# astroHaoPeng/gp_algos

Hardware: AMD Instinct MI355X
Metric: GP posterior (mu,var) points/sec at n=8192 fp64 (fit + predict per step) (higher is better)
Workload: dtype f64; 1 GPU; C2: GP regression, ARD-RBF, n=8192 d=8 fp64, Gram + Cholesky + posterior mean/variance at m=65536 test points per GPU; n=8192, d=8, m_per_gpu=65536, parallelism=single GPU

## Files before the change

gp_algos_amd/csrc/gpcore_api.hip:

```cpp
#include "gpcore_internal.h"

#include <algorithm>
#include <atomic>
#include <queue>
#include <functional>
#include <new>
#include <thread>

void gp_prof_begin(gp_ctx *ctx, int cls, hipStream_t s) {
    if (!(ctx->prof_which & (1 << cls))) return;
    hipEvent_t e0, e1;
    if (hipEventCreate(&e0) != hipSuccess || hipEventCreate(&e1) != hipSuccess) return;
    (void)hipEventRecord(e0, s ? s : ctx->stream);
    ctx->prof[cls].ev.push_back(e0);
    ctx->prof[cls].ev.push_back(e1);
}
void gp_prof_end(gp_ctx *ctx, int cls, double work, hipStream_t s) {
    if (!(ctx->prof_which & (1 << cls))) return;
    gp_prof_slot &p = ctx->prof[cls];
    if (p.ev.size() < 2) return;
    (void)hipEventRecord(p.ev.back(), s ? s : ctx->stream);
    p.launches += 1;
    p.work += work;
}
// ... 368 lines not shown
        const double tiles128 = trapezoid_flops(rows - c1, nnext, wcols) / (2.0 * GP_NB * GP_NB * wcols);
        if (count == 1 && tiles128 < small_update_tiles() && small_panel_update())
            gpk_gemm_k128_sub(s, rows - c1, nnext, P, lda, P, lda, A + (size_t)c1 + (size_t)c1 * lda, lda, 1, wcols);
        else
            gpk_gemm_nt(s, rows - c1, nnext, wcols, -1.0, P, lda, P, lda, 1.0, A + (size_t)c1 + (size_t)c1 * lda, lda, 1, 0, bgemm);
        gp_prof_end(ctx, GP_PROF_SYRK, count * trapezoid_flops(rows - c1, nnext, wcols));
    }
    if (side_busy) (void)hipStreamWaitEvent(s, ctx->ev_b, 0);
}

void back_solve_vec(gp_ctx *ctx, const double *L, int np, int ldl, const double *dinv, double *z, double *alpha) {
    hipStream_t s = ctx->stream;
    for (int k = np / GP_NB - 1; k >= 0; --k)
        gpk_bwd_step(s, L, ldl, dinv + (size_t)k * GP_NB * 16, z, alpha, k * GP_NB);
}

int rows_left_min() {
    const char *e = getenv("GPCORE_ROWS_LEFT_MIN");
    const int x = e ? atoi(e) : 0;
    return x > 0 ? x : 192;
}

void build_lw(gp_ctx *ctx, double *Lw, double *scratch, const double *L, int np, int ldl, const double *dinv) {
    hipStream_t s = ctx->stream;
    gpk_lw_transpose(s, scratch, np, L, ldl, np, 1);
    gp_batch bt;
    bt.count = np / GP_NB;
    bt.s0 = (size_t)GP_NB * np;
    bt.s1 = (size_t)GP_NB * (ldl + 1);
    bt.s2 = (size_t)GP_NB * 16;
    bt.tri = 1;
    gp_prof_begin(ctx, GP_PROF_TRSM);
    gpk_trsm_panel128(s, scratch, np, np, L, ldl, dinv, nullptr, nullptr, nullptr, bt);
    gp_prof_end(ctx, GP_PROF_TRSM, (double)np * np / 2.0 * GP_NB);
    gpk_lw_transpose(s, Lw, np, scratch, np, np, 0);
}

void solve_rows_lower(gp_ctx *ctx, double *Vt, int mp, const double *L, int np, int ldl, const double *dinv, double *sumsq,
                      const double *tvec = nullptr, double *dots = nullptr, const double *Lw = nullptr) {
    hipStream_t s = ctx->stream;
    const int nblk = np / GP_NB;
    if (Lw && sumsq && (mp / GP_NB) >= rows_left_min()) {
        for (int i = 0; i < nblk; ++i) {
            const int K = (i + 1) * GP_NB;
            gp_prof_begin(ctx, GP_PROF_GEMM);
            gpk_gemm_nt_rowred(s, mp, GP_NB, K, Vt, mp, Lw + (size_t)i * GP_NB, np, Vt + (size_t)i * GP_NB * mp, mp, sumsq,
                               tvec ? tvec + (size_t)i * GP_NB : nullptr, dots);
            gp_prof_end(ctx, GP_PROF_GEMM, 2.0 * mp * GP_NB * (double)K);
        }
        return;
    }
    const bool right_looking = (mp / GP_NB) < rows_left_min();
    if (right_looking) {
        const int ob_env = gp_env_blocks("GPCORE_ROWS_OUTER");
        const int OB = ob_env ? ob_env : 2 * GP_OUTER;
        for (int c0 = 0; c0 < np; c0 += OB) {
            const int c1 = std::min(np, c0 + OB);
            for (int k0 = c0; k0 < c1; k0 += GP_NB) {
                double *Vk = Vt + (size_t)k0 * mp;
                gp_prof_begin(ctx, GP_PROF_TRSM);
                gpk_trsm_panel128(s, Vk, mp, mp, L + (size_t)k0 + (size_t)k0 * ldl, ldl, dinv + (size_t)(k0 / GP_NB) * GP_NB * 16, sumsq,
                                  tvec ? tvec + k0 : nullptr, dots);
                gp_prof_end(ctx, GP_PROF_TRSM, (double)mp * GP_NB * GP_NB);
                const int rest = c1 - (k0 + GP_NB);
                if (rest > 0) {
                    gp_prof_begin(ctx, GP_PROF_GEMM);
                    gemm_sub_single(s, mp, rest, GP_NB, Vk, mp, L + (size_t)(k0 + GP_NB) + (size_t)k0 * ldl, ldl, Vt + (size_t)(k0 + GP_NB) * mp, mp);
                    gp_prof_end(ctx, GP_PROF_GEMM, 2.0 * mp * (double)rest * GP_NB);
                }
            }
// ... 266 lines not shown
        if (stream) { ctx->stream = static_cast<hipStream_t>(stream); ctx->own_stream = false; }
        else { e = hipStreamCreateWithFlags(&ctx->stream, hipStreamNonBlocking); ctx->own_stream = true; }
    }
    if (e == hipSuccess) {
        int reserved = 32;
        if (const char *rc = getenv("GPCORE_RESERVED_CUS")) reserved = atoi(rc);
        hipError_t em = hipErrorInvalidValue;
        if (reserved > 0 && ctx->num_cu >= 64) {
            const int words = (ctx->num_cu + 31) / 32;
            std::vector<uint32_t> mask(words, 0xFFFFFFFFu);
            if (ctx->num_cu % 32) mask[words - 1] = (1u << (ctx->num_cu % 32)) - 1u;
            for (int i = 0; i < reserved && i < ctx->num_cu; ++i) mask[i / 32] &= ~(1u << (i % 32));
            em = hipExtStreamCreateWithCUMask(&ctx->side, (uint32_t)words, mask.data());
        }
        if (em != hipSuccess) { (void)hipGetLastError(); e = hipStreamCreateWithFlags(&ctx->side, hipStreamNonBlocking); }
    }
    if (e == hipSuccess && !g_child_ctx && gpi_ctx_ep_streams(ctx) != GP_OK) e = hipErrorInvalidValue;
    if (e == hipSuccess) e = hipEventCreateWithFlags(&ctx->ev_a, hipEventDisableTiming);
    if (e == hipSuccess) e = hipEventCreateWithFlags(&ctx->ev_b, hipEventDisableTiming);
    if (const char *la = getenv("GPCORE_LOOKAHEAD")) ctx->lookahead = atoi(la) != 0 ? 1 : 0;
    if (e == hipSuccess) e = hipMalloc(&ctx->d_scalars, sizeof(double) * 256);
    if (e == hipSuccess) e = hipMalloc(&ctx->d_info, sizeof(int) * 8 + sizeof(double) * 64);
    if (e == hipSuccess) e = hipMemset(ctx->d_info, 0, sizeof(int) * 8 + sizeof(double) * 64);
    if (e == hipSuccess && (gpk_init_diag_kernels() != 0 || gpk_init_gemm_kernels() != 0)) e = hipErrorInvalidValue;
    if (e != hipSuccess) { delete ctx; return GP_EHIP; }
    *out = ctx;
    return GP_OK;
}

void gp_ctx_destroy(gp_ctx *ctx) {
    if (!ctx) return;
    (void)hipSetDevice(ctx->device);
    (void)hipStreamSynchronize(ctx->stream);
    for (int c = 0; c < GP_PROF_NCLASSES; ++c)
        for (hipEvent_t e : ctx->prof[c].ev) (void)hipEventDestroy(e);
    ctx_ext *x = ext_of(ctx);
    for (gp_ctx *c : x->children) gp_ctx_destroy(c);
    x->children.clear();
    (void)hipSetDevice(ctx->device);
    for (int i = 0; i < WS_COUNT; ++i) if (x->ws[i].p) (void)hipFree(x->ws[i].p);
    if (x->mega.d_tasks) (void)hipFree(x->mega.d_tasks);
    if (x->mega.d_done) (void)hipFree(x->mega.d_done);
    if (x->mega.d_ctl) (void)hipFree(x->mega.d_ctl);
    if (x->mega.d_sums) (void)hipFree(x->mega.d_sums);
    if (ctx->d_scalars) (void)hipFree(ctx->d_scalars);
    if (ctx->d_info) (void)hipFree(ctx->d_info);
    if (ctx->ev_a) (void)hipEventDestroy(ctx->ev_a);
// ... 423 lines not shown
    double *Vt, *partial, *sumsq;
    GP_TRY(ws_get(ctx, WS_VT, sizeof(double) * (size_t)mp * np, &Vt));
    GP_TRY(ws_get(ctx, WS_PARTIAL, sizeof(double) * (size_t)nchunk * mp, &partial));
    GP_TRY(ws_get(ctx, WS_SUMSQ, sizeof(double) * (size_t)mp, &sumsq));
    if (np > n) gpk_fill(s, Vt + (size_t)n * mp, (size_t)mp * (np - n), 0.0);
    if (mp > m) {
        GP_HIP(ctx, hipMemset2DAsync(Vt + m, (size_t)mp * 8, 0, (size_t)(mp - m) * 8, n, s));
    }
    gp_prof_begin(ctx, GP_PROF_GRAM);
    if (mdl->kind == 1) gpk_co2_gram(s, dXs, m, mdl->dX, n, mdl->theta.data(), 0, Vt, mp, 0, 1, 0.0);
    else gpk_gram_cross(s, dXs, m, ldxs, mdl->dX, n, n, mdl->d, mdl->theta.data(), Vt, mp, gp_gram_flag(ctx), mdl->dcen);
    gp_prof_end(ctx, GP_PROF_GRAM, 8.0 * m * (double)n + 8.0 * (m + n) * mdl->d);
    double *dots = partial;
    GP_HIP(ctx, hipMemsetAsync(sumsq, 0, sizeof(double) * mp, s));
    GP_HIP(ctx, hipMemsetAsync(dots, 0, sizeof(double) * mp, s));
    const double *Lw = nullptr;
    const bool use_lw = [] { const char *e = getenv("GPCORE_POSTERIOR_LW"); return !e || atoi(e) != 0; }();
    if (use_lw && mp / GP_NB >= rows_left_min()) {
        if (!mdl->dLw) {
            hipError_t e = hipMalloc(&mdl->dLw, sizeof(double) * (size_t)np * np);
            if (e != hipSuccess) { mdl->dLw = nullptr; GP_SET_ERR(ctx, "hipMalloc(Lw, n=%d) failed: %s", n, hipGetErrorString(e)); return GP_ENOMEM; }
        }
        if (!mdl->lw_valid) {
            double *scratch;
            GP_TRY(ws_get(ctx, WS_D, sizeof(double) * (size_t)np * np, &scratch));
            build_lw(ctx, mdl->dLw, scratch, mdl->dL, np, mdl->ldl, mdl->ddinv);
            mdl->lw_valid = true;
        }
        Lw = mdl->dLw;
    }
    solve_rows_lower(ctx, Vt, mp, mdl->dL, np, mdl->ldl, mdl->ddinv, sumsq, mdl->dtmp, dots, Lw);
    GP_HIP(ctx, hipMemcpyAsync(dmean, dots, sizeof(double) * m, hipMemcpyDeviceToDevice, s));
    if (dvar) {
        const double sf = mdl->theta[0], sn = mdl->kind == 1 ? 0.0 : mdl->theta[mdl->d + 1];
        gpk_var_finish(s, dvar, sumsq, m, mdl->kind == 1 ? gpk_co2_kss(mdl->theta.data()) : sf * sf + sn * sn);
    }
    if (vt_out) *vt_out = Vt;
    if (mp_out) *mp_out = mp;
    GP_LAUNCH_CHECK(ctx);
    return GP_OK;
}

static int predict_batch_cap() {
    static const int cap = [] { const char *e = getenv("GPCORE_PREDICT_BATCH"); int v = e ? atoi(e) : 0; return v >= GP_NB ? v / GP_NB * GP_NB : 131072; }();
    return cap;
}

gp_status gp_predict_dev(gp_model *mdl, const double *dXs, int m, int ldxs, double *dmean, double *dvar) {
    if (!mdl) return GP_EINVAL;
// ... 649 lines not shown
```

gp_algos_amd/csrc/gpcore_ep.hip:

```cpp
#include "gpcore_internal.h"
#include "dpp_tile.h"
#include "trsm_tile.h"

#include <algorithm>
#include <atomic>
#include <chrono>
#include <cmath>
#include <new>
#include <thread>
#include <vector>

constexpr int EP_OUTER = 4 * GP_NB;

struct gp_ep {
    gp_ctx *ctx = nullptr;
    int n = 0, np = 0;
    double *K = nullptr;
    double *Sig = nullptr;
    double *Sig2 = nullptr;
    double *L = nullptr;
    int ldl = 0;
    double *dinv = nullptr;
    double *S = nullptr;
    double *Sc = nullptr;
// ... 1385 lines not shown
    GP_REQUIRE(ctx, ep->dX, "classifier was built from a Gram matrix");
    GP_REQUIRE(ctx, dXs && dprob && m >= 0 && ldxs >= m && batch_rows >= 0, "bad arguments");
    GP_REQUIRE(ctx, ep->sweeps > 0, "classifier not trained: run gp_ep_sweep first");
    if (m == 0) return GP_OK;
    GP_HIP(ctx, hipSetDevice(ctx->device));
    hipStream_t s = ctx->stream;
    const int n = ep->n, np = ep->np, d = ep->d;
    int batch = batch_rows > 0 ? std::max(GP_NB, batch_rows / GP_NB * GP_NB)
                               : (int)std::min<size_t>(131072, std::max<size_t>(GP_NB, (((size_t)32 << 30) / ((size_t)np * 8)) / GP_NB * GP_NB));
    batch = std::min(batch, gp_pad(m));
    double *Vt, *partial, *sumsq, *fm;
    GP_TRY(gpi_ws_get(ctx, WS_VT, sizeof(double) * (size_t)batch * np, &Vt));
    GP_TRY(gpi_ws_get(ctx, WS_PARTIAL, sizeof(double) * (size_t)16 * np, &partial));
    GP_TRY(gpi_ws_get(ctx, WS_SUMSQ, sizeof(double) * (size_t)batch, &sumsq));
    GP_TRY(gpi_ws_get(ctx, WS_B, sizeof(double) * (size_t)batch, &fm));
    const double *Lw = nullptr;
    if (batch / GP_NB >= gpi_rows_left_min()) {
        if (!ep->Lw) {
            hipError_t e = hipMalloc(&ep->Lw, sizeof(double) * (size_t)np * np);
            if (e != hipSuccess) { (void)hipGetLastError(); ep->Lw = nullptr; GP_SET_ERR(ctx, "hipMalloc(Lw, n=%d) failed: %s", n, hipGetErrorString(e)); return GP_ENOMEM; }
            ep->lw_valid = false;
        }
        if (!ep->lw_valid) {
            double *scratch;
            GP_TRY(gpi_ws_get(ctx, WS_D, sizeof(double) * (size_t)np * np, &scratch));
            gpi_build_lw(ctx, ep->Lw, scratch, ep->L, np, ep->ldl, ep->dinv);
            ep->lw_valid = true;
        }
        Lw = ep->Lw;
    }
    double *w = ep->tmp2();
    gpk_gemv_rows(s, ep->K, n, n, np, ep->nu(), ep->tmp1(), partial, 16);
    hipLaunchKernelGGL(vec_mul_kernel, g1(n), dim3(256), 0, s, ep->tmp1(), ep->tmp1(), ep->st(), n);
    gpi_forward_solve_vec(ctx, ep->L, np, ep->ldl, ep->dinv, ep->tmp1(), ep->tmp2());
    gpi_back_solve_vec(ctx, ep->L, np, ep->ldl, ep->dinv, ep->tmp2(), ep->tmp1());
    hipLaunchKernelGGL(ep_w_kernel, g1(np), dim3(256), 0, s, w, ep->nu(), ep->st(), ep->tmp1(), n, np);
    const double sf = ep->theta[0], sn = ep->theta[d + 1];
    const double kss = sf * sf + sn * sn;
    for (int lo = 0; lo < m; lo += batch) {
        const int mb = std::min(batch, m - lo), mp = gp_pad(mb);
        gp_prof_begin(ctx, GP_PROF_GRAM);
        gpk_gram_cross(s, dXs + lo, mb, ldxs, ep->dX, n, n, d, ep->theta.data(), Vt, mp, gp_gram_flag(ctx), ep->dcen);
        gp_prof_end(ctx, GP_PROF_GRAM, 8.0 * mb * (double)n + 8.0 * (mb + n) * d);
        hipLaunchKernelGGL(ep_mean_scale_kernel, dim3(mp / GP_NB), dim3(64 * EP_MS_CHUNKS), 0, s, Vt, mp, np, mb, n, w, ep->st(), fm);
        GP_HIP(ctx, hipMemsetAsync(sumsq, 0, sizeof(double) * mp, s));
        gpi_solve_rows_lower(ctx, Vt, mp, ep->L, np, ep->ldl, ep->dinv, sumsq, nullptr, nullptr, Lw);
        hipLaunchKernelGGL(ep_prob_latent_kernel, g1(mb), dim3(256), 0, s, dprob + lo, dfmean ? dfmean + lo : nullptr,
                           dfvar ? dfvar + lo : nullptr, fm, sumsq, kss, mb);
    }
// ... 242 lines not shown
```

gp_algos_amd/csrc/gpcore_internal.h:

```cpp
#pragma once
#include <hip/hip_runtime.h>
#include <cstdint>
#include <cstdio>
#include <cstring>
#include <cstdlib>
#include <cmath>
#include <functional>
#include <vector>

#include "../../include/gpcore.h"

constexpr int GP_NB = 128;
constexpr int GP_BK = 16;
constexpr int GP_OUTER = 512;
static inline int gp_pad(int n) { return (n + GP_NB - 1) / GP_NB * GP_NB; }
static inline int gp_env_blocks(const char *name) {
    const char *e = getenv(name);
    const int v = e ? atoi(e) : 0;
    return (v >= GP_NB && v % GP_NB == 0) ? v : 0;
}

struct gp_prof_slot {
    int64_t launches = 0;
    double work = 0.0;
// ... 45 lines not shown
#define GP_SET_ERR(ctx, ...) do { if (ctx) snprintf((ctx)->err, sizeof((ctx)->err), __VA_ARGS__); } while (0)
#define GP_HIP(ctx, call) do { hipError_t e_ = (call); if (e_ != hipSuccess) { \
    GP_SET_ERR(ctx, "%s:%d %s -> %s", __FILE__, __LINE__, #call, hipGetErrorString(e_)); return GP_EHIP; } } while (0)
#define GP_LAUNCH_CHECK(ctx) GP_HIP(ctx, hipGetLastError())
#define GP_REQUIRE(ctx, cond, msg) do { if (!(cond)) { GP_SET_ERR(ctx, "invalid argument: %s", msg); return GP_EINVAL; } } while (0)
#define GP_TRY(call) do { gp_status s_ = (call); if (s_ != GP_OK) return s_; } while (0)

void gp_prof_begin(gp_ctx *ctx, int cls, hipStream_t s = nullptr);
void gp_prof_end(gp_ctx *ctx, int cls, double work, hipStream_t s = nullptr);

struct gp_batch {
    int count = 1;
    size_t s0 = 0, s1 = 0, s2 = 0;
    size_t s3 = 0, s4 = 0, s5 = 0;
    int tri = 0;
};

void gpk_gemm_nt(hipStream_t s, int M, int N, int K, double alpha, const double *A, int lda, const double *B, int ldb,
                 double beta, double *C, int ldc, int lower, int ktri = 0, gp_batch bt = gp_batch(),
                 const double *Cin = nullptr, int ldcin = 0,
                 int *uflag = nullptr);
void gpk_gemm_k128_sub(hipStream_t s, int M, int N, const double *A, int lda, const double *B, int ldb, double *C, int ldc, int lower, int K = 128);
void gpk_gemm_nt_rowred(hipStream_t s, int M, int N, int K, const double *A, int lda, const double *B, int ldb, double *C, int ldc,
                        double *sumsq, const double *tvec, double *dots);
void gpk_gram_sym(hipStream_t s, const double *X, int n, int d, int ldx, const double *theta, double *K, int ldk, int full, double extra_diag, int *far_flag,
                  const double *center = nullptr);
void gpk_centroid(hipStream_t s, const double *X, int n, int d, int ldx, double *c);
void gpk_dgram_sym(hipStream_t s, const double *X, int n, int d, int ldx, const double *theta, int pos, double *D, int ldd);
void gpk_gram_cross(hipStream_t s, const double *Xs, int m, int ldxs, const double *X, int n, int ldx, int d, const double *theta, double *Ks, int ldks, int *far_flag,
                    const double *center = nullptr);
inline int *gp_gram_flag(gp_ctx *ctx) { return ctx->d_info + 4; }
inline double *gp_gram_center(gp_ctx *ctx) { return reinterpret_cast<double *>(ctx->d_info + 8); }
void gpk_co2_gram(hipStream_t s, const double *xr, int nr, const double *xc, int nc, const double *theta, int pos, double *K, int ldk, int sym,
                  int full, double extra);
void gpk_co2_trace(hipStream_t s, int n, const double *alpha, const double *Kinv, int ldk, const double *D, int ldd, double *partial, double *out);
double gpk_co2_kss(const double *theta);
void gpk_pad_identity(hipStream_t s, double *A, int n, int np, int lda);
void gpk_zero_upper(hipStream_t s, double *A, int n, int lda);
void gpk_fill(hipStream_t s, double *p, size_t count, double v);
void gpk_trsm_panel_upper(hipStream_t s, double *X, int M, int ldx, const double *Ukk, int ldu);
void gpk_transpose(hipStream_t s, double *dst, int ldd, const double *src, int lds, int rows, int cols);
void gpk_lw_transpose(hipStream_t s, double *dst, int ldd, const double *src, int lds, int np, int stage);
void gpk_set_identity(hipStream_t s, double *A, int n, int lda);
void gpk_set_identity_upper(hipStream_t s, double *A, int n, int lda);
void gpk_add_diag(hipStream_t s, double *A, int n, int lda, double v);
void gpk_lml_grad_traces(hipStream_t s, const double *X, int n, int d, int ldx, const double *theta, const double *alpha,
                         const double *Kinv, int ldk, double *partials, double *out);
int gpk_lml_grad_partials_size(int n, int d);
void gpk_gemv_panel_sub(hipStream_t s, const double *A, int M, int lda, const double *x, double *y);
void gpk_gemv_rows(hipStream_t s, const double *Ks, int m, int n, int ldks, const double *alpha, double *out, double *partial, int nchunk, int upper_blocks = 0);
void gpk_lml(hipStream_t s, const double *L, int n, int ldl, const double *t, double *out);
void gpk_var_finish(hipStream_t s, double *var, const double *sumsq, int m, double kss);
size_t gpk_predict_grad_partials(int m, int n, int d);
void gpk_predict_grad(hipStream_t s, const double *Wt, int ldw, const double *Xs, int m, int ldxs, const double *X, int n, int ldx, int d,
                      const double *theta, const double *alpha, double *partials, double *gmean, double *gvar, int ldg);
void gpk_copy_2d(hipStream_t s, double *dst, int ldd, const double *src, int lds, int rows, int cols);
double gpk_probe_mfma(hipStream_t s, int num_cu, int waves_per_simd, double *clock_mhz, double *cycles_per_mfma);
int gpk_init_diag_kernels();
int gpk_init_gemm_kernels();
void gpk_potrf_diag128(hipStream_t s, double *A, int lda, double *dinv_k, int *d_info, int base, gp_batch bt = gp_batch());
void gpk_chol_mega(hipStream_t s, int num_cu, double *A, int lda, double *dinv, int *d_info, const int *tasks, int ntasks, int *done, int *counter,
                   int epoch, int *err, double *sums, unsigned long long *stamps = nullptr);
void gpk_ep_link(hipStream_t s, double *X, int ldx, const double *Lmat, const double *dinv, const double *tvec, double *dots, double *X2,
                 const double *cs2, double *D, int ldd);
void gpk_trsm_panel128(hipStream_t s, double *X, int M, int ldx, const double *Lkk, int ldl, const double *dinv_k, double *sumsq,
                       const double *tvec = nullptr, double *dots = nullptr, gp_batch bt = gp_batch(),
                       double *X2 = nullptr, const double *cs2 = nullptr);
void gpk_fwd_step(hipStream_t s, const double *L, int ldl, const double *dinv_k, double *t, double *sol, int k0, int r);
void gpk_bwd_step(hipStream_t s, const double *L, int ldl, const double *dinv_k, double *t, double *sol, int k0);
void gpk_tile_inverses(hipStream_t s, const double *L, int np, int ldl, double *dinv);
void gpk_copy_strided(hipStream_t s, double *dst, size_t dst_stride, const double *src, size_t src_stride, int count);

enum { WS_VT = 0, WS_PARTIAL, WS_SUMSQ, WS_A, WS_B, WS_C, WS_D, WS_E, WS_F, WS_G, WS_H, WS_COUNT };
gp_status gpi_ws_get(gp_ctx *ctx, int slot, size_t bytes, double **out);
gp_status gpi_upload_2d(gp_ctx *ctx, double *dst, int ldd, const double *src, int lds, int rows, int cols);
gp_status gpi_download_2d(gp_ctx *ctx, double *dst, int ldd, const double *src, int lds, int rows, int cols);
gp_status gpi_read_info(gp_ctx *ctx, int *info);
gp_ctx *gpi_child_ctx(gp_ctx *ctx, int k);
gp_status gpi_model_alpha(gp_model *m, double *dst);
gp_status gpi_model_alloc(gp_ctx *ctx, int n, int d, bool has_x, gp_model **out);
gp_status gpi_lbfgs_maximize(gp_ctx *ctx, int P, int nparams, const double *theta0, int max_iter, int history, int NC,
                             const std::function<gp_status(const double *, int, double *, double *, int *)> &evaluate,
// ... 17 lines not shown
```

gp_algos_amd/csrc/kernels_chol.hip:

```cpp
#include "gpcore_internal.h"

namespace {

constexpr int NB = GP_NB;

__global__ __launch_bounds__(256) void gemv_panel_sub_kernel(const double *__restrict__ A, int M, int lda,
                                                             const double *__restrict__ x, double *__restrict__ y) {
    __shared__ double xs[NB];
    if (threadIdx.x < NB) xs[threadIdx.x] = x[threadIdx.x];
    __syncthreads();
    const int p = blockIdx.x * 256 + threadIdx.x;
    if (p >= M) return;
    double acc = 0.0;
#pragma unroll 8
    for (int k = 0; k < NB; ++k) acc = fma(A[p + (size_t)k * lda], xs[k], acc);
    y[p] -= acc;
}

__global__ __launch_bounds__(256) void gemv_rows_kernel(const double *__restrict__ Ks, int m, int n, int ldks,
                                                        const double *__restrict__ alpha, double *__restrict__ partial,
                                                        int nchunk, int upper_blocks) {
    const int i = blockIdx.x * 256 + threadIdx.x;
    const int ch = blockIdx.y;
    const int per = (n + nchunk - 1) / nchunk;
// ... 61 lines not shown
            for (int c2 = 0; c2 < cc; ++c2) acc[c2] = fma(-x, uc[c2], acc[c2]);
        }
#pragma unroll
        for (int cc = 0; cc < 16; ++cc) xr[(size_t)(cb + cc) * ldx] = acc[cc];
    }
}

__global__ __launch_bounds__(256) void transpose_kernel(double *__restrict__ dst, int ldd, const double *__restrict__ src, int lds,
                                                        int rows, int cols) {
    __shared__ double t[64][65];
    const int r0 = blockIdx.x * 64, c0 = blockIdx.y * 64;
    const int tx = threadIdx.x & 63, ty = threadIdx.x >> 6;
    for (int q = ty; q < 64; q += 4) {
        int r = r0 + tx, c = c0 + q;
        t[q][tx] = (r < rows && c < cols) ? src[r + (size_t)c * lds] : 0.0;
    }
    __syncthreads();
    for (int q = ty; q < 64; q += 4) {
        int c = c0 + tx, r = r0 + q;
        if (r < rows && c < cols) dst[c + (size_t)r * ldd] = t[tx][q];
    }
}

__device__ __forceinline__ void tile_transpose_64(double (*t)[65], double *__restrict__ out, int ldo, int ro, int co,
                                                  const double *__restrict__ in, int ldi, int ri, int ci, double sign) {
    const int tx = threadIdx.x & 63, ty = threadIdx.x >> 6;
    __syncthreads();
    for (int q = ty; q < 64; q += 4) t[q][tx] = in[(ri + tx) + (size_t)(ci + q) * ldi];
    __syncthreads();
    for (int q = ty; q < 64; q += 4) out[(ro + tx) + (size_t)(co + q) * ldo] = sign * t[tx][q];
}
__device__ __forceinline__ void tile_fill_64(double *__restrict__ out, int ldo, int ro, int co, bool identity) {
    const int tx = threadIdx.x & 63, ty = threadIdx.x >> 6;
    for (int q = ty; q < 64; q += 4) out[(ro + tx) + (size_t)(co + q) * ldo] = (identity && tx == q) ? 1.0 : 0.0;
}

__global__ __launch_bounds__(256) void lw_transpose_kernel(double *__restrict__ dst, int ldd, const double *__restrict__ src, int lds, int stage) {
    __shared__ double t[64][65];
    const int ti = blockIdx.x, tj = blockIdx.y;
    if (tj > ti) return;
    const bool same128 = (ti >> 1) == (tj >> 1);
    if (stage) {
        if (!same128) tile_transpose_64(t, dst, ldd, tj * 64, ti * 64, src, lds, ti * 64, tj * 64, -1.0);
        else if (ti == tj) tile_fill_64(dst, ldd, ti * 64, ti * 64, true);
        else { tile_fill_64(dst, ldd, tj * 64, ti * 64, false); tile_fill_64(dst, ldd, ti * 64, tj * 64, false); }
    } else {
        tile_transpose_64(t, dst, ldd, ti * 64, tj * 64, src, lds, tj * 64, ti * 64, 1.0);
        if (same128 && ti != tj) tile_transpose_64(t, dst, ldd, tj * 64, ti * 64, src, lds, ti * 64, tj * 64, 1.0);
    }
}

__global__ void add_diag_kernel(double *A, int n, int lda, double v) {
    const int i = blockIdx.x * blockDim.x + threadIdx.x;
    if (i < n) A[i + (size_t)i * lda] += v;
}
__global__ void set_identity_kernel(double *A, int n, int lda) {
    size_t total = (size_t)n * n;
    for (size_t e = blockIdx.x * (size_t)blockDim.x + threadIdx.x; e < total; e += (size_t)gridDim.x * blockDim.x) {
        int i = (int)(e % n), j = (int)(e / n);
        A[i + (size_t)j * lda] = (i == j) ? 1.0 : 0.0;
    }
}

__global__ void set_identity_upper_kernel(double *A, int n, int lda) {
    for (int j = blockIdx.y; j < n; j += gridDim.y) {
        const int rows = (j & ~127) + 128;
        for (int i = blockIdx.x * blockDim.x + threadIdx.x; i < rows; i += gridDim.x * blockDim.x) A[i + (size_t)j * lda] = (i == j) ? 1.0 : 0.0;
    }
}

constexpr int TR_T = 64, TR_DC = 8, TR_DMAX = 64;
struct TraceParams { double inv_ls2[TR_DMAX]; };
// ... 191 lines not shown
}

struct TraceScale { double s[TR_DMAX + 2]; };
__global__ __launch_bounds__(256) void lml_grad_reduce_kernel(const double *__restrict__ partials, int nblocks, int P, TraceScale sc,
                                                              double *__restrict__ out) {
    __shared__ double red[256];
    const int p = blockIdx.x;
    double acc = 0.0;
    for (int b = threadIdx.x; b < nblocks; b += 256) acc += partials[(size_t)b * P + p];
    double tot = block_sum_256(acc, red);
    if (threadIdx.x == 0) out[p] = sc.s[p] * tot;
}

}

void gpk_trsm_panel_upper(hipStream_t s, double *X, int M, int ldx, const double *Ukk, int ldu) {
    if (M <= 0) return;
    hipLaunchKernelGGL(trsm_panel_upper_kernel, dim3((M + 63) / 64), dim3(64), 0, s, X, M, ldx, Ukk, ldu);
}
void gpk_transpose(hipStream_t s, double *dst, int ldd, const double *src, int lds, int rows, int cols) {
    if (rows <= 0 || cols <= 0) return;
    hipLaunchKernelGGL(transpose_kernel, dim3((rows + 63) / 64, (cols + 63) / 64), dim3(256), 0, s, dst, ldd, src, lds, rows, cols);
}
void gpk_lw_transpose(hipStream_t s, double *dst, int ldd, const double *src, int lds, int np, int stage) {
    hipLaunchKernelGGL(lw_transpose_kernel, dim3(np / 64, np / 64), dim3(256), 0, s, dst, ldd, src, lds, stage);
}
void gpk_add_diag(hipStream_t s, double *A, int n, int lda, double v) {
    if (n > 0) hipLaunchKernelGGL(add_diag_kernel, dim3((n + 255) / 256), dim3(256), 0, s, A, n, lda, v);
}
void gpk_set_identity(hipStream_t s, double *A, int n, int lda) {
    hipLaunchKernelGGL(set_identity_kernel, dim3(1024), dim3(256), 0, s, A, n, lda);
}
void gpk_set_identity_upper(hipStream_t s, double *A, int n, int lda) {
    hipLaunchKernelGGL(set_identity_upper_kernel, dim3(4, n < 65535 ? n : 65535), dim3(256), 0, s, A, n, lda);
}
constexpr int TR_MAX_WG = 768;
int gpk_lml_grad_partials_size(int n, int d) {
    (void)n;
    return TR_MAX_WG * (d + 2);
}
void gpk_lml_grad_traces(hipStream_t s, const double *X, int n, int d, int ldx, const double *theta, const double *alpha,
                         const double *Kinv, int ldk, double *partials, double *out) {
    TraceParams prm;
    TraceScale sc;
    const double sf = theta[0], sn = theta[d + 1];
    for (int k = 0; k < TR_DMAX; ++k) prm.inv_ls2[k] = 0.0;
    for (int k = 0; k < TR_DMAX + 2; ++k) sc.s[k] = 0.0;
    sc.s[0] = sf;
// ... 29 lines not shown
```

gp_algos_amd/csrc/kernels_gemm.hip:

```cpp
#include <type_traits>
#include "gpcore_internal.h"
#include <algorithm>

typedef double double4_t __attribute__((ext_vector_type(4)));
typedef double double2_t __attribute__((ext_vector_type(2)));

namespace {

constexpr int TM = 128, TN = 128, TK = GP_BK;
constexpr int LDS_STRIDE = TM + 16;

__device__ __forceinline__ void tile_coords_lower(int t, int nbm, int nbn, int &bi, int &bj) {
    constexpr int G = 4;
    for (int c0 = 0; c0 < nbn; c0 += G) {
        const int w = (nbn - c0 < G) ? nbn - c0 : G;
        const int head = w * (w + 1) / 2;
        const int total = head + (nbm - c0 - w) * w;
        if (t < total) {
            int r, c;
            if (t < head) {
                r = 0;
                while ((r + 1) * (r + 2) / 2 <= t) ++r;
                c = t - r * (r + 1) / 2;
            } else {
// ... 168 lines not shown
            rsq[mt] += __shfl_xor(rsq[mt], 16, 64);
            rsq[mt] += __shfl_xor(rsq[mt], 32, 64);
            rdt[mt] += __shfl_xor(rdt[mt], 16, 64);
            rdt[mt] += __shfl_xor(rdt[mt], 32, 64);
            if (fk == 0) {
                red[(wave >> 1) * TM + wm + mt * 16 + fr] = rsq[mt];
                red[(NW / 2 + (wave >> 1)) * TM + wm + mt * 16 + fr] = rdt[mt];
            }
        }
        __syncthreads();
        if (tid < TM) {
            double a = 0.0, b = 0.0;
#pragma unroll
            for (int g = 0; g < NW / 2; ++g) { a += red[g * TM + tid]; b += red[(NW / 2 + g) * TM + tid]; }
            rr.sumsq[row0 + tid] += a;
            if (rr.dots) rr.dots[row0 + tid] += b;
        }
    }
}

constexpr int FM = 256, FSTRIDE = FM + 16;
template <int LOWER, int HAS_BETA, int RR, int WV = 16>
__global__ __launch_bounds__(WV * 64, 1) void gemm_fused_kernel(int M, int N, int K, double alpha, const double *A, int lda, const double *B, int ldb,
                                                            double beta, double *C, int ldc, gp_batch bt, gemm_rowred rr) {
    extern __shared__ __attribute__((aligned(16))) double fsm[];
    double *As = fsm;
    double *Bs = fsm + 2 * TK * FSTRIDE;
    const int nbm = M / FM, nbn = N / TN;
    int bi, bj;
    if (LOWER) {
        int t = blockIdx.x;
        bi = 0;
        for (;;) {
            const int cnt = (2 * bi + 2 < nbn) ? 2 * bi + 2 : nbn;
            if (t < cnt) break;
            t -= cnt;
            ++bi;
        }
        bj = t;
    } else {
        const int nwg = gridDim.x, id = blockIdx.x;
        const int q = nwg >> 3, r = nwg & 7, xcd = id & 7;
        const int swz = (xcd < r ? xcd * (q + 1) : r * (q + 1) + (xcd - r) * q) + (id >> 3);
        bi = swz % nbm;
        bj = swz / nbm;
    }
    A += (size_t)blockIdx.y * bt.s0;
// ... 4 lines not shown
    constexpr int NT = (WV == 16) ? 2 : 4;
    const int wm = (wave & 3) * 64, wn = (wave >> 2) * (NT * 16);
    const int fr = lane & 15, fk = lane >> 4;
    const double *Asrc = A + row0 + lane * 2 + (size_t)wave * lda;
    const double *Bsrc = B + col0 + lane * 2 + (size_t)wave * ldb;
    auto stage = [&](int buf, int kt) {
        const size_t koff = (size_t)kt * TK;
#pragma unroll
        for (int q = 0; q < TK / WV; ++q) {
            const int kr = wave + WV * q;
            __builtin_amdgcn_global_load_lds(Asrc + (koff + WV * q) * lda, As + (buf * TK + kr) * FSTRIDE, 16, 0, 0);
            __builtin_amdgcn_global_load_lds(Asrc + 128 + (koff + WV * q) * lda, As + (buf * TK + kr) * FSTRIDE + 128, 16, 0, 0);
            __builtin_amdgcn_global_load_lds(Bsrc + (koff + WV * q) * ldb, Bs + (buf * TK + kr) * LDS_STRIDE, 16, 0, 0);
        }
    };
    double4_t acc[NT][4];
#pragma unroll
    for (int a = 0; a < NT; ++a)
#pragma unroll
        for (int b = 0; b < 4; ++b) acc[a][b] = (double4_t){0.0, 0.0, 0.0, 0.0};
    const int KT = K / TK;
    if (KT > 0) stage(0, 0);
    __syncthreads();
    for (int kt = 0; kt < KT; ++kt) {
        const int cur = kt & 1;
        if (kt + 1 < KT) stage(cur ^ 1, kt + 1);
        const double *Ac = As + cur * TK * FSTRIDE + wm + fr;
        const double *Bc = Bs + cur * TK * LDS_STRIDE + wn + fr;
#pragma unroll
        for (int ks = 0; ks < TK / 4; ++ks) {
            double af[4], bf[NT];
#pragma unroll
            for (int t = 0; t < 4; ++t) af[t] = Ac[(ks * 4 + fk) * FSTRIDE + t * 16];
#pragma unroll
            for (int t = 0; t < NT; ++t) bf[t] = Bc[(ks * 4 + fk) * LDS_STRIDE + t * 16];
#pragma unroll
            for (int nt = 0; nt < NT; ++nt)
#pragma unroll
                for (int mt = 0; mt < 4; ++mt)
                    acc[nt][mt] = __builtin_amdgcn_mfma_f64_16x16x4f64(bf[nt], af[mt], acc[nt][mt], 0, 0, 0);
        }
        __syncthreads();
    }
    const bool diag = LOWER && (row0 < col0 + TN);
    double rsq[4] = {0.0, 0.0, 0.0, 0.0}, rdt[4] = {0.0, 0.0, 0.0, 0.0};
    auto epilogue = [&](auto masked_t) {
        constexpr bool MASKED = decltype(masked_t)::value;
#pragma unroll
        for (int nt = 0; nt < NT; ++nt) {
            double cv[4][4];
            if (HAS_BETA) {
#pragma unroll
                for (int r = 0; r < 4; ++r) {
                    const int n = col0 + wn + nt * 16 + fk + 4 * r;
#pragma unroll
                    for (int mt = 0; mt < 4; ++mt) {
                        const int m = row0 + wm + mt * 16 + fr;
                        cv[r][mt] = (MASKED && m < n) ? 0.0 : C[m + (size_t)n * ldc];
                    }
                }
            }
#pragma unroll
            for (int r = 0; r < 4; ++r) {
                const int n = col0 + wn + nt * 16 + fk + 4 * r;
                const double tn = (RR && rr.dots) ? rr.tvec[n] : 0.0;
// ... 155 lines not shown
    if (uflag) ntiles += 2;
    if (ktri) {
        if (!lower || M != N) return;
        int most = 0;
        for (int x = 0; x < 8; ++x) {
            int cnt = 0;
            for (int r = x; r < M / TM; r += 8) cnt += (r + 1) * bt.count;
            most = cnt > most ? cnt : most;
        }
        ntiles = 8 * most;
        gy = 1;
    }
#define GP_LAUNCH(LO, HB) hipLaunchKernelGGL((gemm_nt_f64_kernel<LO, HB, 8>), dim3(ntiles, gy), dim3(512), 0, s, M, N, K, alpha, A, lda, B, ldb, beta, C, ldc, ktri, bt, rr, Cin, ldcin, uflag)
    if (lower) { if (hb) GP_LAUNCH(1, 1); else GP_LAUNCH(1, 0); }
    else { if (hb) GP_LAUNCH(0, 1); else GP_LAUNCH(0, 0); }
#undef GP_LAUNCH
}

int gpk_init_gemm_kernels() {
    return hipFuncSetAttribute(reinterpret_cast<const void *>(gemm_fused_kernel<0, 0, 1, 8>), hipFuncAttributeMaxDynamicSharedMemorySize, FUSED_LDS) == hipSuccess ? 0 : 1;
}

void gpk_gemm_nt_rowred(hipStream_t s, int M, int N, int K, const double *A, int lda, const double *B, int ldb, double *C, int ldc,
                        double *sumsq, const double *tvec, double *dots) {
    if (M <= 0 || N != TN) return;
    if (M >= FM) {
        static const int ncu = [] { int dev = 0; hipDeviceProp_t pr; return (hipGetDevice(&dev) == hipSuccess && hipGetDeviceProperties(&pr, dev) == hipSuccess && pr.multiProcessorCount > 0) ? pr.multiProcessorCount : 256; }();
        int Mf = M / FM * FM;
        const int rem_tiles = (Mf / FM) % ncu;
        if (Mf / FM > ncu && rem_tiles > 0 && rem_tiles * 2 <= ncu) Mf -= rem_tiles * FM;
        else if (Mf / FM < ncu && Mf / FM * 2 <= ncu / 2) Mf = 0;
        if (Mf == 0) goto small_tiles;
        gemm_rowred r2;
        r2.sumsq = sumsq, r2.tvec = tvec, r2.dots = dots;
        hipLaunchKernelGGL((gemm_fused_kernel<0, 0, 1, 8>), dim3(Mf / FM), dim3(512), FUSED_LDS, s, Mf, TN, K, 1.0, A, lda, B, ldb, 0.0, C, ldc, gp_batch(), r2);
        if (Mf == M) return;
        A += Mf, C += Mf, sumsq += Mf, M -= Mf;
        if (dots) dots += Mf;
    }
small_tiles:
    gemm_rowred rr;
    rr.sumsq = sumsq, rr.tvec = tvec, rr.dots = dots;
    const int ntiles = (M / TM) * (N / TN);
    hipLaunchKernelGGL((gemm_nt_f64_kernel<0, 0, 8, 1>), dim3(ntiles), dim3(512), 0, s, M, N, K, 1.0, A, lda, B, ldb, 0.0, C, ldc, 0, gp_batch(), rr, nullptr, 0, nullptr);
}

void gpk_gemm_k128_sub(hipStream_t s, int M, int N, const double *A, int lda, const double *B, int ldb, double *C, int ldc, int lower, int K) {
    if (M <= 0 || N <= 0 || K <= 0) return;
    const int tm = M / SK_T, tn = N / SK_T;
    if (lower) hipLaunchKernelGGL(gemm_k128_kernel<1>, dim3(tn * tm - tn * (tn - 1) / 2), dim3(256), 0, s, M, N, K, A, lda, B, ldb, C, ldc);
    else hipLaunchKernelGGL(gemm_k128_kernel<0>, dim3(tm * tn), dim3(256), 0, s, M, N, K, A, lda, B, ldb, C, ldc);
}

double gpk_probe_mfma(hipStream_t s, int num_cu, int waves_per_simd, double *clock_mhz, double *cycles_per_mfma) {
    const int iters = 4000;
    const int blocks = num_cu * waves_per_simd;
    double *d = nullptr;
    unsigned long long *st = nullptr;
// ... 26 lines not shown
```

Before: 914,400 points/s.

## Fuse Lw build into one TRSM kernel and skip zero triangle in rowred GEMM

Replaces the transpose, batched TRSM and transpose sequence that builds the inverse-factor matrix Lw with a single kernel. It loads tiles of L (or the identity) into LDS, runs the triangular solve there and writes the transposed result straight to Lw, which drops the scratch buffer and two extra passes over memory. It also passes a triangular flag into the fused row-reduction GEMM so the last diagonal K-tiles skip MFMA work on the zero upper part of the Lw block. This adds per-wave branching in the tail loop and depends on Lw being exactly zero in that region.

```diff
diff --git a/gp_algos_amd/csrc/gpcore_api.hip b/gp_algos_amd/csrc/gpcore_api.hip
--- a/gp_algos_amd/csrc/gpcore_api.hip
+++ b/gp_algos_amd/csrc/gpcore_api.hip
@@ -414,18 +414,10 @@
 }
 
 void build_lw(gp_ctx *ctx, double *Lw, double *scratch, const double *L, int np, int ldl, const double *dinv) {
-    hipStream_t s = ctx->stream;
-    gpk_lw_transpose(s, scratch, np, L, ldl, np, 1);
-    gp_batch bt;
-    bt.count = np / GP_NB;
-    bt.s0 = (size_t)GP_NB * np;
-    bt.s1 = (size_t)GP_NB * (ldl + 1);
-    bt.s2 = (size_t)GP_NB * 16;
-    bt.tri = 1;
+    (void)scratch;
     gp_prof_begin(ctx, GP_PROF_TRSM);
-    gpk_trsm_panel128(s, scratch, np, np, L, ldl, dinv, nullptr, nullptr, nullptr, bt);
+    gpk_build_lw(ctx->stream, Lw, np, L, ldl, dinv, np);
     gp_prof_end(ctx, GP_PROF_TRSM, (double)np * np / 2.0 * GP_NB);
-    gpk_lw_transpose(s, Lw, np, scratch, np, np, 0);
 }
 
 void solve_rows_lower(gp_ctx *ctx, double *Vt, int mp, const double *L, int np, int ldl, const double *dinv, double *sumsq,
@@ -437,7 +429,7 @@
             const int K = (i + 1) * GP_NB;
             gp_prof_begin(ctx, GP_PROF_GEMM);
             gpk_gemm_nt_rowred(s, mp, GP_NB, K, Vt, mp, Lw + (size_t)i * GP_NB, np, Vt + (size_t)i * GP_NB * mp, mp, sumsq,
-                               tvec ? tvec + (size_t)i * GP_NB : nullptr, dots);
+                               tvec ? tvec + (size_t)i * GP_NB : nullptr, dots, 1);
             gp_prof_end(ctx, GP_PROF_GEMM, 2.0 * mp * GP_NB * (double)K);
         }
         return;
@@ -750,7 +742,7 @@
     if (e == hipSuccess) e = hipMalloc(&ctx->d_scalars, sizeof(double) * 256);
     if (e == hipSuccess) e = hipMalloc(&ctx->d_info, sizeof(int) * 8 + sizeof(double) * 64);
     if (e == hipSuccess) e = hipMemset(ctx->d_info, 0, sizeof(int) * 8 + sizeof(double) * 64);
-    if (e == hipSuccess && (gpk_init_diag_kernels() != 0 || gpk_init_gemm_kernels() != 0)) e = hipErrorInvalidValue;
+    if (e == hipSuccess && (gpk_init_diag_kernels() != 0 || gpk_init_gemm_kernels() != 0 || gpk_init_chol_kernels() != 0)) e = hipErrorInvalidValue;
     if (e != hipSuccess) { delete ctx; return GP_EHIP; }
     *out = ctx;
     return GP_OK;
@@ -1220,9 +1212,7 @@
             if (e != hipSuccess) { mdl->dLw = nullptr; GP_SET_ERR(ctx, "hipMalloc(Lw, n=%d) failed: %s", n, hipGetErrorString(e)); return GP_ENOMEM; }
         }
         if (!mdl->lw_valid) {
-            double *scratch;
-            GP_TRY(ws_get(ctx, WS_D, sizeof(double) * (size_t)np * np, &scratch));
-            build_lw(ctx, mdl->dLw, scratch, mdl->dL, np, mdl->ldl, mdl->ddinv);
+            build_lw(ctx, mdl->dLw, nullptr, mdl->dL, np, mdl->ldl, mdl->ddinv);
             mdl->lw_valid = true;
         }
         Lw = mdl->dLw;
diff --git a/gp_algos_amd/csrc/gpcore_ep.hip b/gp_algos_amd/csrc/gpcore_ep.hip
--- a/gp_algos_amd/csrc/gpcore_ep.hip
+++ b/gp_algos_amd/csrc/gpcore_ep.hip
@@ -1431,9 +1431,7 @@
             ep->lw_valid = false;
         }
         if (!ep->lw_valid) {
-            double *scratch;
-            GP_TRY(gpi_ws_get(ctx, WS_D, sizeof(double) * (size_t)np * np, &scratch));
-            gpi_build_lw(ctx, ep->Lw, scratch, ep->L, np, ep->ldl, ep->dinv);
+            gpi_build_lw(ctx, ep->Lw, nullptr, ep->L, np, ep->ldl, ep->dinv);
             ep->lw_valid = true;
         }
         Lw = ep->Lw;
diff --git a/gp_algos_amd/csrc/gpcore_internal.h b/gp_algos_amd/csrc/gpcore_internal.h
--- a/gp_algos_amd/csrc/gpcore_internal.h
+++ b/gp_algos_amd/csrc/gpcore_internal.h
@@ -91,7 +91,7 @@
                  int *uflag = nullptr);
 void gpk_gemm_k128_sub(hipStream_t s, int M, int N, const double *A, int lda, const double *B, int ldb, double *C, int ldc, int lower, int K = 128);
 void gpk_gemm_nt_rowred(hipStream_t s, int M, int N, int K, const double *A, int lda, const double *B, int ldb, double *C, int ldc,
-                        double *sumsq, const double *tvec, double *dots);
+                        double *sumsq, const double *tvec, double *dots, int btri = 0);
 void gpk_gram_sym(hipStream_t s, const double *X, int n, int d, int ldx, const double *theta, double *K, int ldk, int full, double extra_diag, int *far_flag,
                   const double *center = nullptr);
 void gpk_centroid(hipStream_t s, const double *X, int n, int d, int ldx, double *c);
@@ -109,7 +109,7 @@
 void gpk_fill(hipStream_t s, double *p, size_t count, double v);
 void gpk_trsm_panel_upper(hipStream_t s, double *X, int M, int ldx, const double *Ukk, int ldu);
 void gpk_transpose(hipStream_t s, double *dst, int ldd, const double *src, int lds, int rows, int cols);
-void gpk_lw_transpose(hipStream_t s, double *dst, int ldd, const double *src, int lds, int np, int stage);
+void gpk_build_lw(hipStream_t s, double *Lw, int ldw, const double *L, int ldl, const double *dinv, int np);
 void gpk_set_identity(hipStream_t s, double *A, int n, int lda);
 void gpk_set_identity_upper(hipStream_t s, double *A, int n, int lda);
 void gpk_add_diag(hipStream_t s, double *A, int n, int lda, double v);
@@ -127,6 +127,7 @@
 double gpk_probe_mfma(hipStream_t s, int num_cu, int waves_per_simd, double *clock_mhz, double *cycles_per_mfma);
 int gpk_init_diag_kernels();
 int gpk_init_gemm_kernels();
+int gpk_init_chol_kernels();
 void gpk_potrf_diag128(hipStream_t s, double *A, int lda, double *dinv_k, int *d_info, int base, gp_batch bt = gp_batch());
 void gpk_chol_mega(hipStream_t s, int num_cu, double *A, int lda, double *dinv, int *d_info, const int *tasks, int ntasks, int *done, int *counter,
                    int epoch, int *err, double *sums, unsigned long long *stamps = nullptr);
diff --git a/gp_algos_amd/csrc/kernels_chol.hip b/gp_algos_amd/csrc/kernels_chol.hip
--- a/gp_algos_amd/csrc/kernels_chol.hip
+++ b/gp_algos_amd/csrc/kernels_chol.hip
@@ -1,4 +1,5 @@
 #include "gpcore_internal.h"
+#include "trsm_tile.h"
 
 namespace {
 
@@ -107,32 +108,55 @@
     }
 }
 
-__device__ __forceinline__ void tile_transpose_64(double (*t)[65], double *__restrict__ out, int ldo, int ro, int co,
-                                                  const double *__restrict__ in, int ldi, int ri, int ci, double sign) {
-    const int tx = threadIdx.x & 63, ty = threadIdx.x >> 6;
-    __syncthreads();
-    for (int q = ty; q < 64; q += 4) t[q][tx] = in[(ri + tx) + (size_t)(ci + q) * ldi];
-    __syncthreads();
-    for (int q = ty; q < 64; q += 4) out[(ro + tx) + (size_t)(co + q) * ldo] = sign * t[tx][q];
-}
-__device__ __forceinline__ void tile_fill_64(double *__restrict__ out, int ldo, int ro, int co, bool identity) {
-    const int tx = threadIdx.x & 63, ty = threadIdx.x >> 6;
-    for (int q = ty; q < 64; q += 4) out[(ro + tx) + (size_t)(co + q) * ldo] = (identity && tx == q) ? 1.0 : 0.0;
-}
-
-__global__ __launch_bounds__(256) void lw_transpose_kernel(double *__restrict__ dst, int ldd, const double *__restrict__ src, int lds, int stage) {
-    __shared__ double t[64][65];
-    const int ti = blockIdx.x, tj = blockIdx.y;
-    if (tj > ti) return;
-    const bool same128 = (ti >> 1) == (tj >> 1);
-    if (stage) {
-        if (!same128) tile_transpose_64(t, dst, ldd, tj * 64, ti * 64, src, lds, ti * 64, tj * 64, -1.0);
-        else if (ti == tj) tile_fill_64(dst, ldd, ti * 64, ti * 64, true);
-        else { tile_fill_64(dst, ldd, tj * 64, ti * 64, false); tile_fill_64(dst, ldd, ti * 64, tj * 64, false); }
+constexpr int LWS = 65;
+constexpr int LW_LDS = NB * LWS * (int)sizeof(double);
+__global__ __launch_bounds__(256, 2) void build_lw_kernel(double *__restrict__ Lw, int ldw, const double *__restrict__ L, int ldl,
+                                                         const double *__restrict__ dinv) {
+    extern __shared__ __attribute__((aligned(16))) double xs[];
+    const int i = blockIdx.y, k0 = blockIdx.x * 64;
+    if (k0 >= (i + 1) * NB) return;
+    const int tid = threadIdx.x, lane = tid & 63, wave = tid >> 6, fr = lane & 15, fg = lane >> 4;
+    const int c = tid & 127, rh = tid >> 7;
+    if (k0 < i * NB) {
+        const double *src = L + (size_t)i * NB + c + (size_t)(k0 + rh) * ldl;
+#pragma unroll
+        for (int q0 = 0; q0 < 32; q0 += 8) {
+            double v[8];
+#pragma unroll
+            for (int q = 0; q < 8; ++q) v[q] = src[(size_t)(2 * (q0 + q)) * ldl];
+#pragma unroll
+            for (int q = 0; q < 8; ++q) xs[c * LWS + rh + 2 * (q0 + q)] = -1.0 * v[q];
+        }
     } else {
-        tile_transpose_64(t, dst, ldd, ti * 64, tj * 64, src, lds, tj * 64, ti * 64, 1.0);
-        if (same128 && ti != tj) tile_transpose_64(t, dst, ldd, tj * 64, ti * 64, src, lds, ti * 64, tj * 64, 1.0);
-    }
+        const int d0 = k0 - i * NB;
+#pragma unroll 8
+        for (int q = 0; q < 32; ++q) xs[c * LWS + rh + 2 * q] = (c == d0 + rh + 2 * q) ? 1.0 : 0.0;
+    }
+    const double *Ld = L + (size_t)i * NB * ((size_t)ldl + 1), *dv = dinv + (size_t)i * NB * 16;
+    double fa[28], fb[28];
+    trsm_load_frags<1>(Ld, ldl, fr, fg, fa);
+    __syncthreads();
+    const int sp = wave * 16 + fr;
+    double ss = 0.0;
+    trsm_load_frags<2>(Ld, ldl, fr, fg, fb);
+    trsm_chunk<0, LWS>(xs, sp, fr, fg, fa, dv, ss);
+    trsm_chunk<1, LWS>(xs, sp, fr, fg, fa, dv, ss);
+    trsm_load_frags<3>(Ld, ldl, fr, fg, fa);
+    trsm_chunk<2, LWS>(xs, sp, fr, fg, fb, dv, ss);
+    trsm_load_frags<4>(Ld, ldl, fr, fg, fb);
+    trsm_chunk<3, LWS>(xs, sp, fr, fg, fa, dv, ss);
+    trsm_load_frags<5>(Ld, ldl, fr, fg, fa);
+    trsm_chunk<4, LWS>(xs, sp, fr, fg, fb, dv, ss);
+    trsm_load_frags<6>(Ld, ldl, fr, fg, fb);
+    trsm_chunk<5, LWS>(xs, sp, fr, fg, fa, dv, ss);
+    trsm_load_frags<7>(Ld, ldl, fr, fg, fa);
+    trsm_chunk<6, LWS>(xs, sp, fr, fg, fb, dv, ss);
+    trsm_chunk<7, LWS>(xs, sp, fr, fg, fa, dv, ss);
+    (void)ss;
+    __syncthreads();
+    double *dst = Lw + (size_t)i * NB + c + (size_t)(k0 + rh) * ldw;
+#pragma unroll 8
+    for (int q = 0; q < 32; ++q) dst[(size_t)(2 * q) * ldw] = xs[c * LWS + rh + 2 * q];
 }
 
 __global__ void add_diag_kernel(double *A, int n, int lda, double v) {
@@ -370,8 +394,11 @@
     if (rows <= 0 || cols <= 0) return;
     hipLaunchKernelGGL(transpose_kernel, dim3((rows + 63) / 64, (cols + 63) / 64), dim3(256), 0, s, dst, ldd, src, lds, rows, cols);
 }
-void gpk_lw_transpose(hipStream_t s, double *dst, int ldd, const double *src, int lds, int np, int stage) {
-    hipLaunchKernelGGL(lw_transpose_kernel, dim3(np / 64, np / 64), dim3(256), 0, s, dst, ldd, src, lds, stage);
+void gpk_build_lw(hipStream_t s, double *Lw, int ldw, const double *L, int ldl, const double *dinv, int np) {
+    if (np > 0) hipLaunchKernelGGL(build_lw_kernel, dim3(np / 64, np / NB), dim3(256), LW_LDS, s, Lw, ldw, L, ldl, dinv);
+}
+int gpk_init_chol_kernels() {
+    return hipFuncSetAttribute(reinterpret_cast<const void *>(build_lw_kernel), hipFuncAttributeMaxDynamicSharedMemorySize, LW_LDS) == hipSuccess ? 0 : 1;
 }
 void gpk_add_diag(hipStream_t s, double *A, int n, int lda, double v) {
     if (n > 0) hipLaunchKernelGGL(add_diag_kernel, dim3((n + 255) / 256), dim3(256), 0, s, A, n, lda, v);
diff --git a/gp_algos_amd/csrc/kernels_gemm.hip b/gp_algos_amd/csrc/kernels_gemm.hip
--- a/gp_algos_amd/csrc/kernels_gemm.hip
+++ b/gp_algos_amd/csrc/kernels_gemm.hip
@@ -214,7 +214,7 @@
 constexpr int FM = 256, FSTRIDE = FM + 16;
 template <int LOWER, int HAS_BETA, int RR, int WV = 16>
 __global__ __launch_bounds__(WV * 64, 1) void gemm_fused_kernel(int M, int N, int K, double alpha, const double *A, int lda, const double *B, int ldb,
-                                                            double beta, double *C, int ldc, gp_batch bt, gemm_rowred rr) {
+                                                            double beta, double *C, int ldc, gp_batch bt, gemm_rowred rr, int btri) {
     extern __shared__ __attribute__((aligned(16))) double fsm[];
     double *As = fsm;
     double *Bs = fsm + 2 * TK * FSTRIDE;
@@ -265,7 +265,8 @@
     const int KT = K / TK;
     if (KT > 0) stage(0, 0);
     __syncthreads();
-    for (int kt = 0; kt < KT; ++kt) {
+    const int KTF = (btri && NT == 4 && KT >= TN / TK) ? KT - TN / TK : KT;
+    for (int kt = 0; kt < KTF; ++kt) {
         const int cur = kt & 1;
         if (kt + 1 < KT) stage(cur ^ 1, kt + 1);
         const double *Ac = As + cur * TK * FSTRIDE + wm + fr;
@@ -284,6 +285,34 @@
                     acc[nt][mt] = __builtin_amdgcn_mfma_f64_16x16x4f64(bf[nt], af[mt], acc[nt][mt], 0, 0, 0);
         }
         __syncthreads();
+    }
+    if (KTF < KT) {
+        const int wt = __builtin_amdgcn_readfirstlane(wave >> 2) * NT;
+#pragma nounroll
+        for (int kt = KTF; kt < KT; ++kt) {
+            const int cur = kt & 1, skip = (kt - KTF) - wt;
+            if (kt + 1 < KT) stage(cur ^ 1, kt + 1);
+            if (skip < NT) {
+                const double *Ac = As + cur * TK * FSTRIDE + wm + fr;
+                const double *Bc = Bs + cur * TK * LDS_STRIDE + wn + fr;
+#pragma unroll
+                for (int ks = 0; ks < TK / 4; ++ks) {
+                    double af[4];
+#pragma unroll
+                    for (int t = 0; t < 4; ++t) af[t] = Ac[(ks * 4 + fk) * FSTRIDE + t * 16];
+#pragma unroll
+                    for (int nt = 0; nt < NT; ++nt) {
+                        if (nt >= skip) {
+                            const double bf = Bc[(ks * 4 + fk) * LDS_STRIDE + nt * 16];
+#pragma unroll
+                            for (int mt = 0; mt < 4; ++mt)
+                                acc[nt][mt] = __builtin_amdgcn_mfma_f64_16x16x4f64(bf, af[mt], acc[nt][mt], 0, 0, 0);
+                        }
+                    }
+                }
+            }
+            __syncthreads();
+        }
     }
     const bool diag = LOWER && (row0 < col0 + TN);
     double rsq[4] = {0.0, 0.0, 0.0, 0.0}, rdt[4] = {0.0, 0.0, 0.0, 0.0};
@@ -485,7 +514,7 @@
 }
 
 void gpk_gemm_nt_rowred(hipStream_t s, int M, int N, int K, const double *A, int lda, const double *B, int ldb, double *C, int ldc,
-                        double *sumsq, const double *tvec, double *dots) {
+                        double *sumsq, const double *tvec, double *dots, int btri) {
     if (M <= 0 || N != TN) return;
     if (M >= FM) {
         static const int ncu = [] { int dev = 0; hipDeviceProp_t pr; return (hipGetDevice(&dev) == hipSuccess && hipGetDeviceProperties(&pr, dev) == hipSuccess && pr.multiProcessorCount > 0) ? pr.multiProcessorCount : 256; }();
@@ -496,7 +525,7 @@
         if (Mf == 0) goto small_tiles;
         gemm_rowred r2;
         r2.sumsq = sumsq, r2.tvec = tvec, r2.dots = dots;
-        hipLaunchKernelGGL((gemm_fused_kernel<0, 0, 1, 8>), dim3(Mf / FM), dim3(512), FUSED_LDS, s, Mf, TN, K, 1.0, A, lda, B, ldb, 0.0, C, ldc, gp_batch(), r2);
+        hipLaunchKernelGGL((gemm_fused_kernel<0, 0, 1, 8>), dim3(Mf / FM), dim3(512), FUSED_LDS, s, Mf, TN, K, 1.0, A, lda, B, ldb, 0.0, C, ldc, gp_batch(), r2, btri);
         if (Mf == M) return;
         A += Mf, C += Mf, sumsq += Mf, M -= Mf;
         if (dots) dots += Mf;
```

Result: no change. 923,100 points/s (median of 6 runs) (+1.0%).
